# yyl404/NSGP-RePRE

Measured on NVIDIA B200. Metric: nsgp_cov_projection_throughput, higher is better.
Workload: dtype f32 (3xTF32 tensor-core products, fp32 accumulate)

## Files before the change

nsgp-repre_b200/csrc/api.cu:

```cuda
#include <cstdarg>
#include <mutex>
#include <vector>

#include "../../include/nsgp_repre_b200.h"
#include "common.cuh"
#include "geometry.h"
#include "repre.h"
#include "sgd.h"

namespace nsgp {

static thread_local char g_err[512] = "";
unsigned long long g_launches = 0;
#ifdef NSGP_BRINGUP
int g_engine = 0;
#endif

int g_profile = 0;
namespace {
struct ProfRec { cudaEvent_t a, b; };
std::vector<ProfRec> g_prof[kProfKinds];
cudaEvent_t g_prof_open[kProfKinds];
}
namespace {
// ... 1137 lines not shown
               "kmeans_assign: workspace too small");
  size_t n8 = (size_t)round_up(n, 8), k8 = (size_t)round_up(k, 8);
  char* ws = align_up((char*)workspace, 1024);
  float* xh = reinterpret_cast<float*>(ws);
  float* xl = xh + n8 * D;
  float* ch = xl + n8 * D;
  float* cl = ch + k8 * D;
  float* dots = cl + k8 * D;
  int ld = (int)round_up(k, 4);
  float* cn = dots + n8 * ld;
  int rc = launch_split(X, xh, xl, (long long)n * D, stream);
  if (rc) return rc;
  rc = launch_split(centres, ch, cl, (long long)k * D, stream);
  if (rc) return rc;
  rc = launch_row_sqnorm(centres, k, D, D, cn, stream);
  if (rc) return rc;
  NSGP_CHECK_CUDA(cudaMemsetAsync(dots, 0, (size_t)n * ld * 4, stream));
  ContractionArgs a{};
  a.A = matrix_operand(xh, xl, n, D, D);
  a.B = matrix_operand(ch, cl, k, D, D);
  a.out = dots;
  a.ld = ld;
  a.n_cols = k;
  a.alpha = 1.f;
  a.epi = kEpiGemmRmw;
  a.splits = 1;
  rc = contraction(a, stream);
  if (rc) return rc;
  return launch_kmeans_argmin(dots, n, k, ld, cn, (long long*)labels, stream);
}

#ifdef NSGP_BRINGUP
int nsgp_debug_read_counters(unsigned long long* out, int n) {
  NSGP_REQUIRE(out && n != 0 && n <= 160 * 8 && n >= -160 * 8, "debug_read_counters: bad arguments");
  if (n < 0) return debug_read_ac_counters(out, -n);
  return debug_read_counters(out, n);
}

int nsgp_debug_mma_rate(int mode, int iters, unsigned long long* out_dev, int n_ctas,
                        void* stream_) {
  NSGP_REQUIRE(out_dev && iters > 0 && n_ctas > 0, "debug_mma_rate: bad arguments");
  return debug_mma_rate(mode, iters, out_dev, n_ctas, (cudaStream_t)stream_);
}

int nsgp_debug_timeline_read(unsigned long long* out, int* kinds, int max_slots) {
  NSGP_REQUIRE(out && kinds && max_slots > 0, "timeline_read: bad arguments");
  NSGP_CHECK_CUDA(cudaDeviceSynchronize());
  const int n = g_tl_n < max_slots ? g_tl_n : max_slots;
  if (n > 0) {
    NSGP_CHECK_CUDA(cudaMemcpy(out, g_tl_dev, (size_t)n * 2 * sizeof(unsigned long long),
                               cudaMemcpyDeviceToHost));
    for (int i = 0; i < n; ++i) kinds[i] = g_tl_kind[i];
    std::vector<unsigned long long> init(kTlSlots * 2);
    for (int i = 0; i < kTlSlots; ++i) { init[2 * i] = ~0ull; init[2 * i + 1] = 0; }
    cudaMemcpy(g_tl_dev, init.data(), init.size() * sizeof(unsigned long long), cudaMemcpyHostToDevice);
  }
  g_tl_n = 0;
  return n;
}

int nsgp_debug_occupy(int threads, size_t smem, long long cycles, int n_ctas, void* stream_) {
  NSGP_REQUIRE(threads > 0 && threads <= 1024 && n_ctas > 0 && smem <= 227 * 1024,
               "debug_occupy: bad arguments");
  return debug_occupy(threads, smem, cycles, n_ctas, (cudaStream_t)stream_);
}

int nsgp_debug_tma3d_probe(const float* base, long long img_elems, int B, int box_rows,
// ... 45 lines not shown
```

nsgp-repre_b200/csrc/contraction_tc.cu:

```cuda
#include <algorithm>
#include <cstdlib>
#include <mutex>
#include <vector>
#include <unordered_map>

#include "common.cuh"
#include "tc_common.cuh"

namespace nsgp {

using namespace tc;

namespace {

constexpr int BN = 128;
constexpr int STAGES = 3;
constexpr uint32_t kABytes = BM * BK * 4;
constexpr uint32_t kStageBytes = 4 * kABytes;
constexpr uint32_t kTmemCols = 512;

__device__ __forceinline__ int seg_count(int r0, int rows, int br) {
  int n = 0;
  for (int r = r0; r < r0 + BM && r < rows; r += br) ++n;
  return n;
}

struct Item {
  const TcMaps* maps;
  const TcParams* p;
  int rb, cb, kb0, kb1;
};

__device__ __forceinline__ Item fetch_item(const TcMaps* pmaps, const TcParams* pp,
                                           const TcProblem* gprobs, const TcItem* gitems,
                                           int idx) {
  Item it;
  if (gitems != nullptr) {
    const int4 a = *reinterpret_cast<const int4*>(&gitems[idx]);
    const int kb1 = gitems[idx].kb1;
    it.maps = &gprobs[a.x].maps;
    it.p = &gprobs[a.x].p;
    it.rb = a.y; it.cb = a.z; it.kb0 = a.w; it.kb1 = kb1;
    return it;
  }
  it.maps = pmaps;
  it.p = pp;
  const int split = idx / pp->n_tiles;
  int tile = idx - split * pp->n_tiles;
  if (pp->gram) {
    int rb = 0;
    for (;; ++rb) {
      const int cnt = pp->tiles_n - rb;
      if (tile < cnt) break;
      tile -= cnt;
    }
    it.rb = rb; it.cb = rb + tile;
  } else {
    it.rb = tile / pp->tiles_n;
    it.cb = tile - it.rb * pp->tiles_n;
  }
  it.kb0 = (int)((long long)pp->nkb * split / pp->splits);
  it.kb1 = (int)((long long)pp->nkb * (split + 1) / pp->splits);
  return it;
}

__device__ unsigned long long g_dbg_counters[160 * 8];

template <bool PAIR>
__global__ void __launch_bounds__(kThreads, 1)
contraction_tc_kernel(const __grid_constant__ TcMaps pmaps, const __grid_constant__ TcParams pp,
                      const TcProblem* __restrict__ gprobs, const TcItem* __restrict__ gitems,
                      int n_items_max, int prefetch_dist, int dbg,
                      unsigned long long* tl, const int* __restrict__ n_items_dev) {
  const int n_items = n_items_dev != nullptr ? min(n_items_max, __ldg(n_items_dev)) : n_items_max;
  extern __shared__ __align__(1024) uint8_t smem_raw[];
  uint8_t* smem = reinterpret_cast<uint8_t*>(
      (reinterpret_cast<uintptr_t>(smem_raw) + 1023) & ~(uintptr_t)1023);
  uint64_t* full_bar = reinterpret_cast<uint64_t*>(smem + STAGES * kStageBytes);
  uint64_t* empty_bar = full_bar + STAGES;
  uint64_t* tmem_full = empty_bar + STAGES;
  uint64_t* tmem_empty = tmem_full + 2;
  uint64_t* peer_full = tmem_empty + 2;
  uint32_t* tmem_base_slot = reinterpret_cast<uint32_t*>(peer_full + STAGES);

  constexpr int TILE = PAIR ? 256 : 128;
  const int warp = threadIdx.x >> 5;
  const int lane = threadIdx.x & 31;
  const int rank = PAIR ? (int)cluster_ctarank() : 0;
  const int worker = PAIR ? (int)(blockIdx.x >> 1) : (int)blockIdx.x;
  const int n_workers = PAIR ? (int)(gridDim.x >> 1) : (int)gridDim.x;
  const long long t_start = clock64();
  asm volatile("griddepcontrol.launch_dependents;" ::: "memory");
  tl_begin(tl);
  long long c_wait = 0, c_issue = 0, c_acc = 0, c_kb = 0;

  if (warp == 0 && lane == 0) {
    for (int s = 0; s < STAGES; ++s) {
      mbar_init(&full_bar[s], 1);
      mbar_init(&empty_bar[s], 1);
      mbar_init(&peer_full[s], 1);
    }
    for (int b = 0; b < 2; ++b) {
      mbar_init(&tmem_full[b], 1);
      mbar_init(&tmem_empty[b], PAIR ? 8 : 4);
    }
    asm volatile("fence.mbarrier_init.release.cluster;" ::: "memory");
  }
  if (warp == 1) {
    if (PAIR) {
      asm volatile("tcgen05.alloc.cta_group::2.sync.aligned.shared::cta.b32 [%0], %1;" ::"r"(
                       smem_u32(tmem_base_slot)),
                   "r"(kTmemCols)
                   : "memory");
      asm volatile("tcgen05.relinquish_alloc_permit.cta_group::2.sync.aligned;" ::: "memory");
    } else {
      asm volatile("tcgen05.alloc.cta_group::1.sync.aligned.shared::cta.b32 [%0], %1;" ::"r"(
                       smem_u32(tmem_base_slot)),
                   "r"(kTmemCols)
                   : "memory");
      asm volatile("tcgen05.relinquish_alloc_permit.cta_group::1.sync.aligned;" ::: "memory");
    }
  }
  tc_fence_before();
  __syncthreads();
  if (PAIR) cluster_sync();
  tc_fence_after();
  const uint32_t tmem_base = *tmem_base_slot;

  if (warp == 0) {
    uint32_t stage = 0, phase = 0;
    int pf_idx = worker, pf_kb = 0;
    Item pf_it{};
    bool pf_live = prefetch_dist > 0 && pf_idx < n_items;
    if (pf_live) { pf_it = fetch_item(&pmaps, &pp, gprobs, gitems, pf_idx); pf_kb = pf_it.kb0; }
    auto prefetch_step = [&]() {
      if (!pf_live) return;
      const TcParams& q = *pf_it.p;
      const bool pa = q.gram ? (pf_it.rb == pf_it.cb) : (pf_it.cb == 0);
      const bool pb = q.gram ? false : (pf_it.rb == 0);
      const int kx = pf_kb * BK;
      if (pa) {
        const int r0 = pf_it.rb * TILE + rank * BM;
        for (int r = r0; r < r0 + BM && r < q.A.rows; r += q.A.br) {
          const int t = r / q.A.Cs, c = r - t * q.A.Cs;
          const int px = q.A.tile_nkb ? 0 : kx;
          const int py = q.A.tile_nkb ? (((c >> 7) * q.A.tile_nkb + pf_kb) << 7) + (c & 127) : c;
          tma_prefetch_2d_elect(&pf_it.maps->a[0][t], px, py);
          tma_prefetch_2d_elect(&pf_it.maps->a[1][t], px, py);
        }
      }
      if (pb) {
        const int c0 = pf_it.cb * TILE + rank * BM;
        for (int r = c0; r < c0 + BM && r < q.B.rows; r += q.B.br) {
          const int t = r / q.B.Cs, c = r - t * q.B.Cs;
          const int px = q.B.tile_nkb ? 0 : kx;
          const int py = q.B.tile_nkb ? (((c >> 7) * q.B.tile_nkb + pf_kb) << 7) + (c & 127) : c;
          tma_prefetch_2d_elect(&pf_it.maps->b[0][t], px, py);
          tma_prefetch_2d_elect(&pf_it.maps->b[1][t], px, py);
        }
      }
      if (++pf_kb >= pf_it.kb1) {
        pf_idx += n_workers;
        pf_live = pf_idx < n_items;
        if (pf_live) { pf_it = fetch_item(&pmaps, &pp, gprobs, gitems, pf_idx); pf_kb = pf_it.kb0; }
      }
    };
    for (int i = 0; i < prefetch_dist; ++i) prefetch_step();
    for (int idx = worker; idx < n_items; idx += n_workers) {
      const Item it = fetch_item(&pmaps, &pp, gprobs, gitems, idx);
      const TcParams& p = *it.p;
      const int r0 = it.rb * TILE + rank * BM;
      const int c0 = it.cb * TILE + rank * BM;
      const bool share = p.gram && p.same_operand && it.rb == it.cb;
      const int a_rows = p.A.rows, a_br = p.A.br, a_cs = p.A.Cs, a_tn = p.A.tile_nkb;
      const int b_rows = p.B.rows, b_br = p.B.br, b_cs = p.B.Cs, b_tn = p.B.tile_nkb;
      const int segs_a = seg_count(r0, a_rows, a_br);
      const int segs_b = share ? 0 : seg_count(c0, b_rows, b_br);
      const uint32_t tx =
          ((dbg & 4) ? 1u : 2u) * (uint32_t)(segs_a * a_br + segs_b * b_br) * BK * 4u;
      for (int kb = it.kb0; kb < it.kb1; ++kb) {
        prefetch_step();
        long long t0 = (dbg & 1) ? clock64() : 0;
        if (dbg & 8) mbar_wait(&empty_bar[stage], phase ^ 1);
        else mbar_wait_warp(&empty_bar[stage], phase ^ 1, lane);
        long long t1 = (dbg & 1) ? clock64() : 0;
        c_wait += t1 - t0;
        mbar_expect_tx_elect(&full_bar[stage], tx);
        const uint32_t sbase = smem_u32(smem + stage * kStageBytes);
        const int kx0 = kb * BK;
        for (int s = 0; s < segs_a; ++s) {
          const int r = r0 + s * a_br;
          const int t = r / a_cs, c = r - t * a_cs;
          const uint32_t off = (uint32_t)(s * a_br) * (BK * 4);
          const int lx = a_tn ? 0 : kx0;
          const int ly = a_tn ? (((c >> 7) * a_tn + kb) << 7) + (c & 127) : c;
          tma_load_2d_elect(sbase + off, &it.maps->a[0][t], &full_bar[stage], lx, ly);
          if (!(dbg & 4)) tma_load_2d_elect(sbase + kABytes + off, &it.maps->a[1][t], &full_bar[stage], lx, ly);
        }
        for (int s = 0; s < segs_b; ++s) {
          const int r = c0 + s * b_br;
          const int t = r / b_cs, c = r - t * b_cs;
          const uint32_t off = (uint32_t)(s * b_br) * (BK * 4);
          const int lx = b_tn ? 0 : kx0;
          const int ly = b_tn ? (((c >> 7) * b_tn + kb) << 7) + (c & 127) : c;
          tma_load_2d_elect(sbase + 2 * kABytes + off, &it.maps->b[0][t], &full_bar[stage], lx, ly);
          if (!(dbg & 4)) tma_load_2d_elect(sbase + 3 * kABytes + off, &it.maps->b[1][t], &full_bar[stage], lx, ly);
        }
        if (dbg & 1) c_issue += clock64() - t1;
        if (++stage == STAGES) { stage = 0; phase ^= 1; }
      }
    }
    if ((dbg & 1) && lane == 0) {
      g_dbg_counters[blockIdx.x * 8 + 3] = c_wait;
      g_dbg_counters[blockIdx.x * 8 + 4] = c_issue;
    }
  } else if (warp == 1) {
    if (!PAIR || rank == 0) {
      uint32_t stage = 0, phase = 0;
      uint32_t local_item = 0;
      for (int idx = worker; idx < n_items; idx += n_workers, ++local_item) {
        const Item it = fetch_item(&pmaps, &pp, gprobs, gitems, idx);
        const TcParams& p = *it.p;
        const bool share = p.gram && p.same_operand && it.rb == it.cb;
        int n_valid = p.n_cols - it.cb * TILE;
        if (n_valid > TILE) n_valid = TILE;
        const uint32_t idesc = PAIR ? make_idesc_tf32(256, 256)
                                    : make_idesc_tf32(BM, (n_valid + 15) & ~15);
        const uint32_t buf = local_item & 1;
        const uint32_t use = local_item >> 1;
        long long ta = (dbg & 1) ? clock64() : 0;
        mbar_wait_warp(&tmem_empty[buf], (use & 1) ^ 1, lane);
        if (dbg & 1) c_acc += clock64() - ta;
        tc_fence_after();
        const uint32_t d_main = tmem_base + buf * 256;
        const uint32_t d_corr = d_main + 128;
        for (int kb = it.kb0; kb < it.kb1; ++kb) {
          long long t0 = (dbg & 1) ? clock64() : 0;
          if (dbg & 8) mbar_wait(&full_bar[stage], phase);
          else mbar_wait_warp(&full_bar[stage], phase, lane);
          if (PAIR) mbar_wait_warp(&peer_full[stage], phase, lane);
          long long t1 = (dbg & 1) ? clock64() : 0;
          c_wait += t1 - t0;
          ++c_kb;
          tc_fence_after();
          const uint32_t sbase = smem_u32(smem + stage * kStageBytes);
          const uint64_t a_hi = make_kmajor_sw128_desc(sbase);
          const uint64_t a_lo = make_kmajor_sw128_desc(sbase + kABytes);
          const uint64_t b_hi = share ? a_hi : make_kmajor_sw128_desc(sbase + 2 * kABytes);
          const uint64_t b_lo = share ? a_lo : make_kmajor_sw128_desc(sbase + 3 * kABytes);
          const uint32_t first = kb > it.kb0 ? 1u : 0u;
          if (PAIR) {
            tc_mma_kblock_3xtf32_2sm(d_main, a_hi, a_lo, b_hi, b_lo, idesc, first);
            tc_commit_2sm_mc_elect(&empty_bar[stage]);
            if (kb == it.kb1 - 1) tc_commit_2sm_mc_elect(&tmem_full[buf]);
          } else {
            if (dbg & 2) tc_mma_kblock_3xtf32(d_main, d_corr, a_hi, a_hi, b_hi, b_hi, idesc, first, 2u);
            else tc_mma_kblock_3xtf32(d_main, d_corr, a_hi, a_lo, b_hi, b_lo, idesc, first, 0u);
            tc_commit_elect(&empty_bar[stage]);
            if (kb == it.kb1 - 1) tc_commit_elect(&tmem_full[buf]);
          }
          if (dbg & 1) c_issue += clock64() - t1;
          if (++stage == STAGES) { stage = 0; phase ^= 1; }
        }
        if (it.kb1 <= it.kb0) {
          if (PAIR) tc_commit_2sm_mc_elect(&tmem_full[buf]);
          else tc_commit_elect(&tmem_full[buf]);
        }
      }
      if ((dbg & 1) && lane == 0) {
        g_dbg_counters[blockIdx.x * 8 + 0] = c_wait;
        g_dbg_counters[blockIdx.x * 8 + 1] = c_issue;
        g_dbg_counters[blockIdx.x * 8 + 2] = c_acc;
        g_dbg_counters[blockIdx.x * 8 + 5] = clock64() - t_start;
        g_dbg_counters[blockIdx.x * 8 + 6] = c_kb;
      }
    } else {
      uint32_t stage = 0, phase = 0;
      for (int idx = worker; idx < n_items; idx += n_workers) {
        const Item it = fetch_item(&pmaps, &pp, gprobs, gitems, idx);
        for (int kb = it.kb0; kb < it.kb1; ++kb) {
          mbar_wait_warp(&full_bar[stage], phase, lane);
          mbar_arrive_remote_elect(&peer_full[stage], 0);
          if (++stage == STAGES) { stage = 0; phase ^= 1; }
        }
      }
    }
  } else {
    const int quad = warp & 3;
    uint32_t local_item = 0;
    for (int idx = worker; idx < n_items; idx += n_workers, ++local_item) {
      const Item it = fetch_item(&pmaps, &pp, gprobs, gitems, idx);
      const TcParams& p = *it.p;
      const uint32_t buf = local_item & 1;
      const uint32_t use = local_item >> 1;
      mbar_wait_warp(&tmem_full[buf], use & 1, lane, 200);
      tc_fence_after();
      const int rblk = it.rb * TILE + rank * BM;
      const int row = rblk + quad * 32 + lane;
      const bool row_ok = row < p.A.rows && it.kb1 > it.kb0;
      float* orow = p.out + (long long)row * p.ld;
      const float alpha = p.alpha;
      const int n_cols = p.n_cols;
      const bool vec = p.vec_red != 0;
      const bool gram = p.gram != 0;
#pragma unroll 1
      for (int chunk = 0; chunk < TILE / 32; ++chunk) {
        uint32_t v[32];
        const uint32_t taddr = tmem_base + ((uint32_t)(quad * 32) << 16) + buf * 256 + chunk * 32;
        tc_ld32(taddr, v);
        if (!PAIR) {
          uint32_t w[32];
          tc_ld32(taddr + 128, w);
          tc_wait_ld();
#pragma unroll
          for (int j = 0; j < 32; ++j)
            v[j] = __float_as_uint(__uint_as_float(v[j]) + __uint_as_float(w[j]));
        } else {
          tc_wait_ld();
        }
        const int col0 = it.cb * TILE + chunk * 32;
        const bool wanted = !gram || (col0 + 31 >= rblk);
        if (row_ok && col0 < n_cols && wanted) {
#pragma unroll
          for (int j = 0; j < 32; j += 4) {
            const int col = col0 + j;
            const float x0 = alpha * __uint_as_float(v[j]), x1 = alpha * __uint_as_float(v[j + 1]),
                        x2 = alpha * __uint_as_float(v[j + 2]), x3 = alpha * __uint_as_float(v[j + 3]);
            if (vec && col + 3 < n_cols) {
              red_add_v4(orow + col, x0, x1, x2, x3);
            } else {
              if (col < n_cols) atomicAdd(orow + col, x0);
              if (col + 1 < n_cols) atomicAdd(orow + col + 1, x1);
              if (col + 2 < n_cols) atomicAdd(orow + col + 2, x2);
              if (col + 3 < n_cols) atomicAdd(orow + col + 3, x3);
            }
          }
        }
      }
      tc_fence_before();
      __syncwarp();
      if (!PAIR || rank == 0) {
        if (lane == 0) mbar_arrive(&tmem_empty[buf]);
      } else {
        mbar_arrive_remote_elect(&tmem_empty[buf], 0);
      }
    }
  }

  tc_fence_before();
  __syncthreads();
  tl_end(tl);
  if (PAIR) cluster_sync();
  if (warp == 1) {
    tc_fence_after();
    if (PAIR)
      asm volatile("tcgen05.dealloc.cta_group::2.sync.aligned.b32 %0, %1;" ::"r"(tmem_base),
                   "r"(kTmemCols)
                   : "memory");
    else
      asm volatile("tcgen05.dealloc.cta_group::1.sync.aligned.b32 %0, %1;" ::"r"(tmem_base),
                   "r"(kTmemCols)
                   : "memory");
  }
}

typedef CUresult (*EncodeTiledFn)(CUtensorMap*, CUtensorMapDataType, cuuint32_t, void*,
                                  const cuuint64_t*, const cuuint64_t*, const cuuint32_t*,
                                  const cuuint32_t*, CUtensorMapInterleave, CUtensorMapSwizzle,
                                  CUtensorMapL2promotion, CUtensorMapFloatOOBfill);

EncodeTiledFn get_encode_fn() {
  static EncodeTiledFn fn = nullptr;
  static std::once_flag once;
  std::call_once(once, [] {
    void* p = nullptr;
    cudaDriverEntryPointQueryResult q;
    if (cudaGetDriverEntryPoint("cuTensorMapEncodeTiled", &p, cudaEnableDefault, &q) ==
            cudaSuccess &&
        q == cudaDriverEntryPointSuccess)
      fn = reinterpret_cast<EncodeTiledFn>(p);
  });
  return fn;
}

int pick_box_rows(const Operand& o) {
  if (o.T == 1) {
    int br = 128;
    while (br > o.Cs) br >>= 1;
    return br < 8 ? 0 : br;
  }
  for (int br = 128; br >= 8; br >>= 1)
    if (o.Cs % br == 0) return br;
  return 0;
}

int encode_operand(const Operand& o, int br, CUtensorMap (*dst)[kMaxTaps]) {
  EncodeTiledFn enc = get_encode_fn();
  NSGP_REQUIRE(enc != nullptr, "tcgen05 engine: cuTensorMapEncodeTiled is unavailable");
  for (int hl = 0; hl < 2; ++hl)
    for (int t = 0; t < o.T; ++t) {
      const float* base = o.base + (long long)hl * o.hl_stride + o.tap_off[t];
      NSGP_REQUIRE((reinterpret_cast<uintptr_t>(base) & 15) == 0,
                   "tcgen05 engine: operand base must be 16-byte aligned");
      cuuint64_t gdim[2] = {(cuuint64_t)o.K, (cuuint64_t)o.Cs};
      cuuint64_t gstr[1] = {(cuuint64_t)o.row_pitch * 4};
      if (o.tile_nkb > 0) {
        gdim[0] = BK;
        gdim[1] = (cuuint64_t)ceil_div(o.Cs, 128) * o.tile_nkb * 128;
        gstr[0] = BK * 4;
      }
      cuuint32_t box[2] = {(cuuint32_t)BK, (cuuint32_t)br};
      cuuint32_t estr[2] = {1, 1};
      CUresult r = enc(&dst[hl][t], CU_TENSOR_MAP_DATA_TYPE_FLOAT32, 2, (void*)base, gdim, gstr,
                       box, estr, CU_TENSOR_MAP_INTERLEAVE_NONE, CU_TENSOR_MAP_SWIZZLE_128B,
                       CU_TENSOR_MAP_L2_PROMOTION_L2_256B, CU_TENSOR_MAP_FLOAT_OOB_FILL_NONE);
      NSGP_REQUIRE(r == CUDA_SUCCESS,
                   "cuTensorMapEncodeTiled failed (%d): K=%d Cs=%d pitch=%lld br=%d", (int)r, o.K,
                   o.Cs, o.row_pitch, br);
    }
  return 0;
}

void fill_operand(const Operand& o, int br, TcOperand* d) {
  d->T = o.T; d->Cs = o.Cs; d->rows = o.rows; d->br = br;
  d->tile_nkb = o.tile_nkb; d->pad0 = d->pad1 = d->pad2 = 0;
}

constexpr size_t kSmemBytes = (size_t)STAGES * kStageBytes + 1024 + 256;
constexpr size_t kSmemBytesFullSm = (size_t)7 * 32768 + 1024 + 256;

int dbg_counters() {
  static const int d = (nsgp_env("NSGP_DBG_COUNTERS") ? 1 : 0) | (nsgp_env("NSGP_DBG_MMA2") ? 2 : 0) |
                       (nsgp_env("NSGP_DBG_HALFLOAD") ? 4 : 0) | (nsgp_env("NSGP_DBG_ALLPOLL") ? 8 : 0);
  return d;
}

int prefetch_distance() {
  static const int d = [] {
    const char* e = nsgp_env("NSGP_PREFETCH");
    return e ? atoi(e) : 8;
  }();
  return d;
}

template <bool PAIR>
int configure_kernel() {
  static bool configured = false;
// ... 95 lines not shown
  NSGP_REQUIRE(br_a > 0 && br_b > 0, "tcgen05 engine: operand rows per tap must be >= 8 "
               "(multiple of 8 when taps > 1)");
  TcParams& p = out->p;
  p = TcParams{};
  p.nkb = k_blocks(a.A);
  if (a.A.rows == 0 || a.n_cols == 0 || p.nkb == 0) return 1;
  int rc = encode_operand(a.A, br_a, out->maps.a);
  if (rc) return rc;
  rc = encode_operand(a.B, br_b, out->maps.b);
  if (rc) return rc;
  fill_operand(a.A, br_a, &p.A);
  fill_operand(a.B, br_b, &p.B);
  p.out = a.out; p.ld = a.ld; p.n_cols = a.n_cols; p.alpha = a.alpha;
  p.gram = (a.epi == kEpiGramAtomic) ? 1 : 0;
  p.same_operand = (p.gram && a.A.base == a.B.base && a.A.hl_stride == a.B.hl_stride &&
                    a.A.rows == a.B.rows) ? 1 : 0;
  p.pair = pair ? 1 : 0;
  p.chain = a.chain;
  const int tile = pair ? 256 : 128;
  p.tiles_m = ceil_div(a.A.rows, tile);
  p.tiles_n = ceil_div(a.n_cols, tile);
  NSGP_REQUIRE(!p.gram || p.tiles_m == p.tiles_n, "Gram: operands must have the same rows");
  p.n_tiles = p.gram ? p.tiles_m * (p.tiles_m + 1) / 2 : p.tiles_m * p.tiles_n;
  static const int vec_red = [] {
    const char* e = nsgp_env("NSGP_VEC_RED");
    return (e && e[0] == '0') ? 0 : 1;
  }();
  p.vec_red = (vec_red && a.ld % 4 == 0 && (reinterpret_cast<uintptr_t>(a.out) & 15) == 0) ? 1 : 0;
  p.splits = 1;
  return 0;
}

int chain_limit(const TcParams& p) {
  static const int gram_chain = [] {
    const char* e = nsgp_env("NSGP_CHAIN");
    return e ? atoi(e) : kChainGram;
  }();
  if (p.chain > 0) return p.pair && p.chain > 32 ? 32 : p.chain;
  if (!p.gram) return kChainGemm;
  return p.pair ? 32 : gram_chain;
}

}

int encode_batch_rows_map(CUtensorMap* dst, const float* base, long long img_elems, int B,
                          int box_rows) {
  EncodeTiledFn enc = get_encode_fn();
  NSGP_REQUIRE(enc != nullptr, "cuTensorMapEncodeTiled is unavailable");
  NSGP_REQUIRE(img_elems % 256 == 0 && (reinterpret_cast<uintptr_t>(base) & 15) == 0,
               "batch rows map: input must be 16-byte aligned with a multiple of 256 elements");
  cuuint64_t gdim[3] = {256, (cuuint64_t)(img_elems / 256), (cuuint64_t)B};
  cuuint64_t gstr[2] = {1024, (cuuint64_t)img_elems * 4};
  cuuint32_t box[3] = {256, (cuuint32_t)box_rows, (cuuint32_t)B};
  cuuint32_t estr[3] = {1, 1, 1};
  CUresult r = enc(dst, CU_TENSOR_MAP_DATA_TYPE_FLOAT32, 3, (void*)base, gdim, gstr, box, estr,
                   CU_TENSOR_MAP_INTERLEAVE_NONE, CU_TENSOR_MAP_SWIZZLE_NONE,
                   CU_TENSOR_MAP_L2_PROMOTION_L2_256B, CU_TENSOR_MAP_FLOAT_OOB_FILL_NONE);
  NSGP_REQUIRE(r == CUDA_SUCCESS, "cuTensorMapEncodeTiled (batch rows) failed (%d)", (int)r);
  return 0;
}

namespace tc {
int sm_count() {
  static int n = 0;
  if (n == 0) {
    int dev = 0;
    cudaGetDevice(&dev);
    cudaDeviceGetAttribute(&n, cudaDevAttrMultiProcessorCount, dev);
    if (n <= 0) n = 148;
  }
  return n;
}
}
// ... 164 lines not shown
```

nsgp-repre_b200/csrc/tc_common.cuh:

```cuda
#pragma once
#include "common.cuh"

namespace nsgp {
namespace tc {

constexpr int BM = 128;
constexpr int BK = 32;
constexpr int UMMA_K = 8;
constexpr int kThreads = 192;
constexpr int kEpiWarp0 = 2;

struct alignas(64) TcMaps {
  CUtensorMap a[2][kMaxTaps];
  CUtensorMap b[2][kMaxTaps];
};

struct TcOperand {
  int T, Cs, rows, br;
  int tile_nkb, pad0, pad1, pad2;
};

struct TcParams {
  TcOperand A, B;
  float* out;
// ... 91 lines not shown
      "tcgen05.mma.cta_group::1.kind::tf32 [%0], %1, %2, %3, p;\n\t}" ::"r"(d_tmem),
      "l"(adesc), "l"(bdesc), "r"(idesc), "r"(accumulate)
      : "memory");
}
__device__ __forceinline__ void tc_ld32(uint32_t taddr, uint32_t (&v)[32]) {
  asm volatile(
      "tcgen05.ld.sync.aligned.32x32b.x32.b32 "
      "{%0, %1, %2, %3, %4, %5, %6, %7, %8, %9, %10, %11, %12, %13, %14, %15, "
      "%16, %17, %18, %19, %20, %21, %22, %23, %24, %25, %26, %27, %28, %29, %30, %31}, [%32];"
      : "=r"(v[0]), "=r"(v[1]), "=r"(v[2]), "=r"(v[3]), "=r"(v[4]), "=r"(v[5]), "=r"(v[6]),
        "=r"(v[7]), "=r"(v[8]), "=r"(v[9]), "=r"(v[10]), "=r"(v[11]), "=r"(v[12]), "=r"(v[13]),
        "=r"(v[14]), "=r"(v[15]), "=r"(v[16]), "=r"(v[17]), "=r"(v[18]), "=r"(v[19]),
        "=r"(v[20]), "=r"(v[21]), "=r"(v[22]), "=r"(v[23]), "=r"(v[24]), "=r"(v[25]),
        "=r"(v[26]), "=r"(v[27]), "=r"(v[28]), "=r"(v[29]), "=r"(v[30]), "=r"(v[31])
      : "r"(taddr)
      : "memory");
}
__device__ __forceinline__ void tc_wait_ld() {
  asm volatile("tcgen05.wait::ld.sync.aligned;" ::: "memory");
}
__device__ __forceinline__ void red_add_v4(float* p, float a, float b, float c, float d) {
  asm volatile("red.global.add.v4.f32 [%0], {%1, %2, %3, %4};" ::"l"(p), "f"(a), "f"(b),
               "f"(c), "f"(d)
               : "memory");
}

__device__ __forceinline__ uint64_t make_kmajor_sw128_desc(uint32_t saddr) {
  uint64_t d = 0;
  d |= (uint64_t)((saddr >> 4) & 0x3FFF);
  d |= (uint64_t)1 << 16;
  d |= (uint64_t)(1024 >> 4) << 32;
  d |= (uint64_t)1 << 46;
  d |= (uint64_t)2 << 61;
  return d;
}

__host__ __device__ constexpr uint32_t make_idesc_tf32(int M, int N) {
  return (1u << 4) | (2u << 7) | (2u << 10) | ((uint32_t)(N >> 3) << 17) |
         ((uint32_t)(M >> 4) << 24);
}


__device__ __forceinline__ void mbar_expect_tx_elect(uint64_t* bar, uint32_t bytes) {
  asm volatile(
      "{\n\t.reg .pred pe;\n\t"
      "elect.sync _|pe, 0xffffffff;\n\t"
      "@pe mbarrier.arrive.expect_tx.shared::cta.b64 _, [%0], %1;\n\t}" ::"r"(smem_u32(bar)),
      "r"(bytes)
      : "memory");
}
__device__ __forceinline__ void tma_load_2d_elect(uint32_t dst, const CUtensorMap* map,
                                                  uint64_t* bar, int x, int c) {
  asm volatile(
      "{\n\t.reg .pred pe;\n\t"
      "elect.sync _|pe, 0xffffffff;\n\t"
      "@pe cp.async.bulk.tensor.2d.shared::cluster.global.tile.mbarrier::complete_tx::bytes "
      "[%0], [%1, {%3, %4}], [%2];\n\t}" ::"r"(dst),
      "l"(reinterpret_cast<uint64_t>(map)), "r"(smem_u32(bar)), "r"(x), "r"(c)
      : "memory");
}
__device__ __forceinline__ void tc_commit_elect(uint64_t* bar) {
  asm volatile(
      "{\n\t.reg .pred pe;\n\t"
      "elect.sync _|pe, 0xffffffff;\n\t"
      "@pe tcgen05.commit.cta_group::1.mbarrier::arrive::one.shared::cluster.b64 [%0];\n\t}" ::
      "r"(smem_u32(bar))
// ... 8 lines not shown
      ".reg .pred pe, pf, pc, pt;\n\t"
      "setp.eq.b32 pt, 0, 0;\n\t"
      ".reg .b64 ah, al, bh, bl;\n\t"
      "elect.sync _|pe, 0xffffffff;\n\t"
      "setp.ne.b32 pf, %7, 0;\n\t"
      "setp.eq.b32 pc, %8, 1;\n\t"
      "or.pred pc, pc, pf;\n\t"
      ".reg .pred ps, pq;\n\t"
      "setp.lt.u32 ps, %8, 2;\n\t"
      "and.pred ps, ps, pe;\n\t"
      "setp.ne.b32 pq, %8, 3;\n\t"
      "and.pred pq, pq, pe;\n\t"
      "@pe tcgen05.mma.cta_group::1.kind::tf32 [%0], %2, %4, %6, pf;\n\t"
      "@pq tcgen05.mma.cta_group::1.kind::tf32 [%1], %3, %4, %6, pc;\n\t"
      "@ps tcgen05.mma.cta_group::1.kind::tf32 [%1], %2, %5, %6, pt;\n\t"
      "add.u64 ah, %2, 2; add.u64 al, %3, 2; add.u64 bh, %4, 2; add.u64 bl, %5, 2;\n\t"
      "@pe tcgen05.mma.cta_group::1.kind::tf32 [%0], ah, bh, %6, pt;\n\t"
      "@pq tcgen05.mma.cta_group::1.kind::tf32 [%1], al, bh, %6, pt;\n\t"
      "@ps tcgen05.mma.cta_group::1.kind::tf32 [%1], ah, bl, %6, pt;\n\t"
      "add.u64 ah, %2, 4; add.u64 al, %3, 4; add.u64 bh, %4, 4; add.u64 bl, %5, 4;\n\t"
      "@pe tcgen05.mma.cta_group::1.kind::tf32 [%0], ah, bh, %6, pt;\n\t"
      "@pq tcgen05.mma.cta_group::1.kind::tf32 [%1], al, bh, %6, pt;\n\t"
      "@ps tcgen05.mma.cta_group::1.kind::tf32 [%1], ah, bl, %6, pt;\n\t"
      "add.u64 ah, %2, 6; add.u64 al, %3, 6; add.u64 bh, %4, 6; add.u64 bl, %5, 6;\n\t"
      "@pe tcgen05.mma.cta_group::1.kind::tf32 [%0], ah, bh, %6, pt;\n\t"
      "@pq tcgen05.mma.cta_group::1.kind::tf32 [%1], al, bh, %6, pt;\n\t"
      "@ps tcgen05.mma.cta_group::1.kind::tf32 [%1], ah, bl, %6, pt;\n\t"
      "}" ::"r"(d_main),
      "r"(d_corr), "l"(a_hi), "l"(a_lo), "l"(b_hi), "l"(b_lo), "r"(idesc), "r"(first),
      "r"(same_acc)
      : "memory");
}

__device__ __forceinline__ void tc_cp_a_kblock(uint32_t t_hi, uint32_t t_lo, uint64_t a_hi,
                                               uint64_t a_lo) {
  asm volatile(
      "{\n\t.reg .pred pe;\n\t.reg .b64 ah, al;\n\t"
      "elect.sync _|pe, 0xffffffff;\n\t"
      "@pe tcgen05.cp.cta_group::1.128x256b [%0], %2;\n\t"
      "@pe tcgen05.cp.cta_group::1.128x256b [%1], %3;\n\t"
      "add.u64 ah, %2, 2; add.u64 al, %3, 2;\n\t"
      "@pe tcgen05.cp.cta_group::1.128x256b [%0 + 8], ah;\n\t"
      "@pe tcgen05.cp.cta_group::1.128x256b [%1 + 8], al;\n\t"
      "add.u64 ah, %2, 4; add.u64 al, %3, 4;\n\t"
      "@pe tcgen05.cp.cta_group::1.128x256b [%0 + 16], ah;\n\t"
      "@pe tcgen05.cp.cta_group::1.128x256b [%1 + 16], al;\n\t"
      "add.u64 ah, %2, 6; add.u64 al, %3, 6;\n\t"
      "@pe tcgen05.cp.cta_group::1.128x256b [%0 + 24], ah;\n\t"
      "@pe tcgen05.cp.cta_group::1.128x256b [%1 + 24], al;\n\t"
      "}" ::"r"(t_hi), "r"(t_lo), "l"(a_hi), "l"(a_lo)
      : "memory");
}
__device__ __forceinline__ void tc_mma_kblock_3xtf32_ta(uint32_t d, uint32_t t_hi, uint32_t t_lo,
                                                        uint64_t b_hi, uint64_t b_lo,
                                                        uint32_t idesc, uint32_t first) {
  asm volatile(
      "{\n\t"
      ".reg .pred pe, pf, pt;\n\t"
      ".reg .b64 bh, bl;\n\t"
      "setp.eq.b32 pt, 0, 0;\n\t"
      "elect.sync _|pe, 0xffffffff;\n\t"
      "setp.ne.b32 pf, %6, 0;\n\t"
      "@pe tcgen05.mma.cta_group::1.kind::tf32 [%0], [%1], %3, %5, pf;\n\t"
      "@pe tcgen05.mma.cta_group::1.kind::tf32 [%0], [%2], %3, %5, pt;\n\t"
      "@pe tcgen05.mma.cta_group::1.kind::tf32 [%0], [%1], %4, %5, pt;\n\t"
      "add.u64 bh, %3, 2; add.u64 bl, %4, 2;\n\t"
// ... 42 lines not shown
      "r"(rank)
      : "memory");
}
__device__ __forceinline__ void tc_mma_kblock_3xtf32_2sm(uint32_t d, uint64_t a_hi, uint64_t a_lo,
                                                         uint64_t b_hi, uint64_t b_lo,
                                                         uint32_t idesc, uint32_t first) {
  asm volatile(
      "{\n\t"
      ".reg .pred pe, pf, pt;\n\t"
      ".reg .b64 ah, al, bh, bl;\n\t"
      "setp.eq.b32 pt, 0, 0;\n\t"
      "elect.sync _|pe, 0xffffffff;\n\t"
      "setp.ne.b32 pf, %6, 0;\n\t"
      "@pe tcgen05.mma.cta_group::2.kind::tf32 [%0], %2, %3, %5, pf;\n\t"
      "@pe tcgen05.mma.cta_group::2.kind::tf32 [%0], %1, %4, %5, pt;\n\t"
      "@pe tcgen05.mma.cta_group::2.kind::tf32 [%0], %1, %3, %5, pt;\n\t"
      "add.u64 ah, %1, 2; add.u64 al, %2, 2; add.u64 bh, %3, 2; add.u64 bl, %4, 2;\n\t"
      "@pe tcgen05.mma.cta_group::2.kind::tf32 [%0], al, bh, %5, pt;\n\t"
      "@pe tcgen05.mma.cta_group::2.kind::tf32 [%0], ah, bl, %5, pt;\n\t"
      "@pe tcgen05.mma.cta_group::2.kind::tf32 [%0], ah, bh, %5, pt;\n\t"
      "add.u64 ah, %1, 4; add.u64 al, %2, 4; add.u64 bh, %3, 4; add.u64 bl, %4, 4;\n\t"
      "@pe tcgen05.mma.cta_group::2.kind::tf32 [%0], al, bh, %5, pt;\n\t"
      "@pe tcgen05.mma.cta_group::2.kind::tf32 [%0], ah, bl, %5, pt;\n\t"
      "@pe tcgen05.mma.cta_group::2.kind::tf32 [%0], ah, bh, %5, pt;\n\t"
      "add.u64 ah, %1, 6; add.u64 al, %2, 6; add.u64 bh, %3, 6; add.u64 bl, %4, 6;\n\t"
      "@pe tcgen05.mma.cta_group::2.kind::tf32 [%0], al, bh, %5, pt;\n\t"
      "@pe tcgen05.mma.cta_group::2.kind::tf32 [%0], ah, bl, %5, pt;\n\t"
      "@pe tcgen05.mma.cta_group::2.kind::tf32 [%0], ah, bh, %5, pt;\n\t"
      "}" ::"r"(d),
      "l"(a_hi), "l"(a_lo), "l"(b_hi), "l"(b_lo), "r"(idesc), "r"(first)
      : "memory");
}

__device__ __forceinline__ void tma_prefetch_2d_elect(const CUtensorMap* map, int x, int c) {
  asm volatile(
      "{\n\t.reg .pred pe;\n\t"
      "elect.sync _|pe, 0xffffffff;\n\t"
      "@pe cp.async.bulk.prefetch.tensor.2d.L2.global.tile [%0, {%1, %2}];\n\t}" ::"l"(
          reinterpret_cast<uint64_t>(map)),
      "r"(x), "r"(c)
      : "memory");
}

constexpr uint32_t kPeerBitMask = 0xFEFFFFFFu;
__device__ __forceinline__ uint32_t cluster_ctarank() {
  uint32_t r;
  asm volatile("mov.u32 %0, %%cluster_ctarank;" : "=r"(r));
  return r;
}
__device__ __forceinline__ void cluster_sync() {
  asm volatile("barrier.cluster.arrive.release.aligned;" ::: "memory");
  asm volatile("barrier.cluster.wait.acquire.aligned;" ::: "memory");
}
__device__ __forceinline__ void mbar_arrive_remote(uint64_t* bar, uint32_t rank) {
  asm volatile(
      "{\n\t.reg .b32 ra;\n\t"
      "mapa.shared::cluster.u32 ra, %0, %1;\n\t"
      "mbarrier.arrive.release.cluster.shared::cluster.b64 _, [ra];\n\t}" ::"r"(smem_u32(bar)),
      "r"(rank)
      : "memory");
}
__device__ __forceinline__ void tma_load_2d_2sm(uint32_t dst, const CUtensorMap* map,
                                                uint64_t* bar, int x, int c) {
  asm volatile(
      "cp.async.bulk.tensor.2d.cta_group::2.shared::cluster.global.mbarrier::complete_tx::bytes "
      "[%0], [%1, {%3, %4}], [%2];" ::"r"(dst),
// ... 27 lines not shown
```

Measured before the change: 433.1.

## Split k-blocks into half-width SW64 stages and deepen pipeline to seven

```diff
diff --git a/nsgp-repre_b200/csrc/api.cu b/nsgp-repre_b200/csrc/api.cu
--- a/nsgp-repre_b200/csrc/api.cu
+++ b/nsgp-repre_b200/csrc/api.cu
@@ -1193,7 +1193,7 @@
 
 #ifdef NSGP_BRINGUP
 int nsgp_debug_read_counters(unsigned long long* out, int n) {
-  NSGP_REQUIRE(out && n != 0 && n <= 160 * 8 && n >= -160 * 8, "debug_read_counters: bad arguments");
+  NSGP_REQUIRE(out && n != 0 && n <= 2 * 160 * 8 && n >= -160 * 8, "debug_read_counters: bad arguments");
   if (n < 0) return debug_read_ac_counters(out, -n);
   return debug_read_counters(out, n);
 }
diff --git a/nsgp-repre_b200/csrc/contraction_tc.cu b/nsgp-repre_b200/csrc/contraction_tc.cu
--- a/nsgp-repre_b200/csrc/contraction_tc.cu
+++ b/nsgp-repre_b200/csrc/contraction_tc.cu
@@ -14,8 +14,10 @@
 namespace {
 
 constexpr int BN = 128;
-constexpr int STAGES = 3;
-constexpr uint32_t kABytes = BM * BK * 4;
+constexpr int SUB = 2;
+constexpr int BKS = BK / SUB;
+constexpr int STAGES = 7;
+constexpr uint32_t kABytes = BM * BKS * 4;
 constexpr uint32_t kStageBytes = 4 * kABytes;
 constexpr uint32_t kTmemCols = 512;
 
@@ -64,7 +66,7 @@
   return it;
 }
 
-__device__ unsigned long long g_dbg_counters[160 * 8];
+__device__ unsigned long long g_dbg_counters[2 * 160 * 8];
 
 template <bool PAIR>
 __global__ void __launch_bounds__(kThreads, 1)
@@ -73,6 +75,9 @@
                       int n_items_max, int prefetch_dist, int dbg,
                       unsigned long long* tl, const int* __restrict__ n_items_dev) {
   const int n_items = n_items_dev != nullptr ? min(n_items_max, __ldg(n_items_dev)) : n_items_max;
+#ifndef NSGP_BRINGUP
+  dbg = 0;
+#endif
   extern __shared__ __align__(1024) uint8_t smem_raw[];
   uint8_t* smem = reinterpret_cast<uint8_t*>(
       (reinterpret_cast<uintptr_t>(smem_raw) + 1023) & ~(uintptr_t)1023);
@@ -92,7 +97,7 @@
   const long long t_start = clock64();
   asm volatile("griddepcontrol.launch_dependents;" ::: "memory");
   tl_begin(tl);
-  long long c_wait = 0, c_issue = 0, c_acc = 0, c_kb = 0;
+  long long c_wait = 0, c_issue = 0, c_acc = 0, c_kb = 0, c_peer = 0;
 
   if (warp == 0 && lane == 0) {
     for (int s = 0; s < STAGES; ++s) {
@@ -145,8 +150,10 @@
           const int t = r / q.A.Cs, c = r - t * q.A.Cs;
           const int px = q.A.tile_nkb ? 0 : kx;
           const int py = q.A.tile_nkb ? (((c >> 7) * q.A.tile_nkb + pf_kb) << 7) + (c & 127) : c;
-          tma_prefetch_2d_elect(&pf_it.maps->a[0][t], px, py);
-          tma_prefetch_2d_elect(&pf_it.maps->a[1][t], px, py);
+          for (int h = 0; h < SUB; ++h) {
+            tma_prefetch_2d_elect(&pf_it.maps->a[0][t], px + h * BKS, py);
+            tma_prefetch_2d_elect(&pf_it.maps->a[1][t], px + h * BKS, py);
+          }
         }
       }
       if (pb) {
@@ -155,8 +162,10 @@
           const int t = r / q.B.Cs, c = r - t * q.B.Cs;
           const int px = q.B.tile_nkb ? 0 : kx;
           const int py = q.B.tile_nkb ? (((c >> 7) * q.B.tile_nkb + pf_kb) << 7) + (c & 127) : c;
-          tma_prefetch_2d_elect(&pf_it.maps->b[0][t], px, py);
-          tma_prefetch_2d_elect(&pf_it.maps->b[1][t], px, py);
+          for (int h = 0; h < SUB; ++h) {
+            tma_prefetch_2d_elect(&pf_it.maps->b[0][t], px + h * BKS, py);
+            tma_prefetch_2d_elect(&pf_it.maps->b[1][t], px + h * BKS, py);
+          }
         }
       }
       if (++pf_kb >= pf_it.kb1) {
@@ -177,9 +186,10 @@
       const int segs_a = seg_count(r0, a_rows, a_br);
       const int segs_b = share ? 0 : seg_count(c0, b_rows, b_br);
       const uint32_t tx =
-          ((dbg & 4) ? 1u : 2u) * (uint32_t)(segs_a * a_br + segs_b * b_br) * BK * 4u;
-      for (int kb = it.kb0; kb < it.kb1; ++kb) {
-        prefetch_step();
+          ((dbg & 4) ? 1u : 2u) * (uint32_t)(segs_a * a_br + segs_b * b_br) * BKS * 4u;
+      for (int j = it.kb0 * SUB; j < it.kb1 * SUB; ++j) {
+        const int kb = j / SUB, h = j - kb * SUB;
+        if (h == 0) prefetch_step();
         long long t0 = (dbg & 1) ? clock64() : 0;
         if (dbg & 8) mbar_wait(&empty_bar[stage], phase ^ 1);
         else mbar_wait_warp(&empty_bar[stage], phase ^ 1, lane);
@@ -187,12 +197,12 @@
         c_wait += t1 - t0;
         mbar_expect_tx_elect(&full_bar[stage], tx);
         const uint32_t sbase = smem_u32(smem + stage * kStageBytes);
-        const int kx0 = kb * BK;
+        const int kx0 = kb * BK + h * BKS;
         for (int s = 0; s < segs_a; ++s) {
           const int r = r0 + s * a_br;
           const int t = r / a_cs, c = r - t * a_cs;
-          const uint32_t off = (uint32_t)(s * a_br) * (BK * 4);
-          const int lx = a_tn ? 0 : kx0;
+          const uint32_t off = (uint32_t)(s * a_br) * (BKS * 4);
+          const int lx = a_tn ? h * BKS : kx0;
           const int ly = a_tn ? (((c >> 7) * a_tn + kb) << 7) + (c & 127) : c;
           tma_load_2d_elect(sbase + off, &it.maps->a[0][t], &full_bar[stage], lx, ly);
           if (!(dbg & 4)) tma_load_2d_elect(sbase + kABytes + off, &it.maps->a[1][t], &full_bar[stage], lx, ly);
@@ -200,8 +210,8 @@
         for (int s = 0; s < segs_b; ++s) {
           const int r = c0 + s * b_br;
           const int t = r / b_cs, c = r - t * b_cs;
-          const uint32_t off = (uint32_t)(s * b_br) * (BK * 4);
-          const int lx = b_tn ? 0 : kx0;
+          const uint32_t off = (uint32_t)(s * b_br) * (BKS * 4);
+          const int lx = b_tn ? h * BKS : kx0;
           const int ly = b_tn ? (((c >> 7) * b_tn + kb) << 7) + (c & 127) : c;
           tma_load_2d_elect(sbase + 2 * kABytes + off, &it.maps->b[0][t], &full_bar[stage], lx, ly);
           if (!(dbg & 4)) tma_load_2d_elect(sbase + 3 * kABytes + off, &it.maps->b[1][t], &full_bar[stage], lx, ly);
@@ -234,30 +244,33 @@
         tc_fence_after();
         const uint32_t d_main = tmem_base + buf * 256;
         const uint32_t d_corr = d_main + 128;
-        for (int kb = it.kb0; kb < it.kb1; ++kb) {
+        for (int j = it.kb0 * SUB; j < it.kb1 * SUB; ++j) {
           long long t0 = (dbg & 1) ? clock64() : 0;
           if (dbg & 8) mbar_wait(&full_bar[stage], phase);
           else mbar_wait_warp(&full_bar[stage], phase, lane);
+          long long tp = (dbg & 1) ? clock64() : 0;
           if (PAIR) mbar_wait_warp(&peer_full[stage], phase, lane);
           long long t1 = (dbg & 1) ? clock64() : 0;
-          c_wait += t1 - t0;
-          ++c_kb;
+          c_wait += tp - t0;
+          c_peer += t1 - tp;
+          if (j % SUB == 0) ++c_kb;
           tc_fence_after();
           const uint32_t sbase = smem_u32(smem + stage * kStageBytes);
-          const uint64_t a_hi = make_kmajor_sw128_desc(sbase);
-          const uint64_t a_lo = make_kmajor_sw128_desc(sbase + kABytes);
-          const uint64_t b_hi = share ? a_hi : make_kmajor_sw128_desc(sbase + 2 * kABytes);
-          const uint64_t b_lo = share ? a_lo : make_kmajor_sw128_desc(sbase + 3 * kABytes);
-          const uint32_t first = kb > it.kb0 ? 1u : 0u;
+          const uint64_t a_hi = make_kmajor_sw64_desc(sbase);
+          const uint64_t a_lo = make_kmajor_sw64_desc(sbase + kABytes);
+          const uint64_t b_hi = share ? a_hi : make_kmajor_sw64_desc(sbase + 2 * kABytes);
+          const uint64_t b_lo = share ? a_lo : make_kmajor_sw64_desc(sbase + 3 * kABytes);
+          const uint32_t first = j > it.kb0 * SUB ? 1u : 0u;
+          const bool last = j == it.kb1 * SUB - 1;
           if (PAIR) {
-            tc_mma_kblock_3xtf32_2sm(d_main, a_hi, a_lo, b_hi, b_lo, idesc, first);
+            tc_mma_half_3xtf32_2sm(d_main, a_hi, a_lo, b_hi, b_lo, idesc, first);
             tc_commit_2sm_mc_elect(&empty_bar[stage]);
-            if (kb == it.kb1 - 1) tc_commit_2sm_mc_elect(&tmem_full[buf]);
+            if (last) tc_commit_2sm_mc_elect(&tmem_full[buf]);
           } else {
-            if (dbg & 2) tc_mma_kblock_3xtf32(d_main, d_corr, a_hi, a_hi, b_hi, b_hi, idesc, first, 2u);
-            else tc_mma_kblock_3xtf32(d_main, d_corr, a_hi, a_lo, b_hi, b_lo, idesc, first, 0u);
+            if (dbg & 2) tc_mma_half_3xtf32(d_main, d_corr, a_hi, a_hi, b_hi, b_hi, idesc, first, 2u);
+            else tc_mma_half_3xtf32(d_main, d_corr, a_hi, a_lo, b_hi, b_lo, idesc, first, 0u);
             tc_commit_elect(&empty_bar[stage]);
-            if (kb == it.kb1 - 1) tc_commit_elect(&tmem_full[buf]);
+            if (last) tc_commit_elect(&tmem_full[buf]);
           }
           if (dbg & 1) c_issue += clock64() - t1;
           if (++stage == STAGES) { stage = 0; phase ^= 1; }
@@ -273,12 +286,13 @@
         g_dbg_counters[blockIdx.x * 8 + 2] = c_acc;
         g_dbg_counters[blockIdx.x * 8 + 5] = clock64() - t_start;
         g_dbg_counters[blockIdx.x * 8 + 6] = c_kb;
+        g_dbg_counters[blockIdx.x * 8 + 7] = c_peer;
       }
     } else {
       uint32_t stage = 0, phase = 0;
       for (int idx = worker; idx < n_items; idx += n_workers) {
         const Item it = fetch_item(&pmaps, &pp, gprobs, gitems, idx);
-        for (int kb = it.kb0; kb < it.kb1; ++kb) {
+        for (int j = it.kb0 * SUB; j < it.kb1 * SUB; ++j) {
           mbar_wait_warp(&full_bar[stage], phase, lane);
           mbar_arrive_remote_elect(&peer_full[stage], 0);
           if (++stage == STAGES) { stage = 0; phase ^= 1; }
@@ -293,7 +307,10 @@
       const TcParams& p = *it.p;
       const uint32_t buf = local_item & 1;
       const uint32_t use = local_item >> 1;
+      const long long te0 = (dbg & 1) ? clock64() : 0;
       mbar_wait_warp(&tmem_full[buf], use & 1, lane, 200);
+      const long long te1 = (dbg & 1) ? clock64() : 0;
+      c_wait += te1 - te0;
       tc_fence_after();
       const int rblk = it.rb * TILE + rank * BM;
       const int row = rblk + quad * 32 + lane;
@@ -344,6 +361,11 @@
       } else {
         mbar_arrive_remote_elect(&tmem_empty[buf], 0);
       }
+      if (dbg & 1) c_issue += clock64() - te1;
+    }
+    if ((dbg & 1) && warp == kEpiWarp0 && lane == 0) {
+      g_dbg_counters[160 * 8 + blockIdx.x * 8 + 0] = c_wait;
+      g_dbg_counters[160 * 8 + blockIdx.x * 8 + 1] = c_issue;
     }
   }
 
@@ -409,10 +431,10 @@
         gdim[1] = (cuuint64_t)ceil_div(o.Cs, 128) * o.tile_nkb * 128;
         gstr[0] = BK * 4;
       }
-      cuuint32_t box[2] = {(cuuint32_t)BK, (cuuint32_t)br};
+      cuuint32_t box[2] = {(cuuint32_t)BKS, (cuuint32_t)br};
       cuuint32_t estr[2] = {1, 1};
       CUresult r = enc(&dst[hl][t], CU_TENSOR_MAP_DATA_TYPE_FLOAT32, 2, (void*)base, gdim, gstr,
-                       box, estr, CU_TENSOR_MAP_INTERLEAVE_NONE, CU_TENSOR_MAP_SWIZZLE_128B,
+                       box, estr, CU_TENSOR_MAP_INTERLEAVE_NONE, CU_TENSOR_MAP_SWIZZLE_64B,
                        CU_TENSOR_MAP_L2_PROMOTION_L2_256B, CU_TENSOR_MAP_FLOAT_OOB_FILL_NONE);
       NSGP_REQUIRE(r == CUDA_SUCCESS,
                    "cuTensorMapEncodeTiled failed (%d): K=%d Cs=%d pitch=%lld br=%d", (int)r, o.K,
@@ -574,13 +596,14 @@
 }
 
 int chain_limit(const TcParams& p) {
-  static const int gram_chain = [] {
+  static const int chain_env = [] {
     const char* e = nsgp_env("NSGP_CHAIN");
-    return e ? atoi(e) : kChainGram;
+    return e ? atoi(e) : 0;
   }();
   if (p.chain > 0) return p.pair && p.chain > 32 ? 32 : p.chain;
   if (!p.gram) return kChainGemm;
-  return p.pair ? 32 : gram_chain;
+  if (chain_env > 0) return chain_env;
+  return p.pair ? 32 : kChainGram;
 }
 
 }
diff --git a/nsgp-repre_b200/csrc/tc_common.cuh b/nsgp-repre_b200/csrc/tc_common.cuh
--- a/nsgp-repre_b200/csrc/tc_common.cuh
+++ b/nsgp-repre_b200/csrc/tc_common.cuh
@@ -147,6 +147,16 @@
   d |= (uint64_t)(1024 >> 4) << 32;
   d |= (uint64_t)1 << 46;
   d |= (uint64_t)2 << 61;
+  return d;
+}
+
+__device__ __forceinline__ uint64_t make_kmajor_sw64_desc(uint32_t saddr) {
+  uint64_t d = 0;
+  d |= (uint64_t)((saddr >> 4) & 0x3FFF);
+  d |= (uint64_t)1 << 16;
+  d |= (uint64_t)(512 >> 4) << 32;
+  d |= (uint64_t)1 << 46;
+  d |= (uint64_t)4 << 61;
   return d;
 }
 
@@ -221,6 +231,37 @@
       : "memory");
 }
 
+__device__ __forceinline__ void tc_mma_half_3xtf32(uint32_t d_main, uint32_t d_corr,
+                                                   uint64_t a_hi, uint64_t a_lo, uint64_t b_hi,
+                                                   uint64_t b_lo, uint32_t idesc,
+                                                   uint32_t first, uint32_t same_acc) {
+  asm volatile(
+      "{\n\t"
+      ".reg .pred pe, pf, pc, pt;\n\t"
+      "setp.eq.b32 pt, 0, 0;\n\t"
+      ".reg .b64 ah, al, bh, bl;\n\t"
+      "elect.sync _|pe, 0xffffffff;\n\t"
+      "setp.ne.b32 pf, %7, 0;\n\t"
+      "setp.eq.b32 pc, %8, 1;\n\t"
+      "or.pred pc, pc, pf;\n\t"
+      ".reg .pred ps, pq;\n\t"
+      "setp.lt.u32 ps, %8, 2;\n\t"
+      "and.pred ps, ps, pe;\n\t"
+      "setp.ne.b32 pq, %8, 3;\n\t"
+      "and.pred pq, pq, pe;\n\t"
+      "@pe tcgen05.mma.cta_group::1.kind::tf32 [%0], %2, %4, %6, pf;\n\t"
+      "@pq tcgen05.mma.cta_group::1.kind::tf32 [%1], %3, %4, %6, pc;\n\t"
+      "@ps tcgen05.mma.cta_group::1.kind::tf32 [%1], %2, %5, %6, pt;\n\t"
+      "add.u64 ah, %2, 2; add.u64 al, %3, 2; add.u64 bh, %4, 2; add.u64 bl, %5, 2;\n\t"
+      "@pe tcgen05.mma.cta_group::1.kind::tf32 [%0], ah, bh, %6, pt;\n\t"
+      "@pq tcgen05.mma.cta_group::1.kind::tf32 [%1], al, bh, %6, pt;\n\t"
+      "@ps tcgen05.mma.cta_group::1.kind::tf32 [%1], ah, bl, %6, pt;\n\t"
+      "}" ::"r"(d_main),
+      "r"(d_corr), "l"(a_hi), "l"(a_lo), "l"(b_hi), "l"(b_lo), "r"(idesc), "r"(first),
+      "r"(same_acc)
+      : "memory");
+}
+
 __device__ __forceinline__ void tc_cp_a_kblock(uint32_t t_hi, uint32_t t_lo, uint64_t a_hi,
                                                uint64_t a_lo) {
   asm volatile(
@@ -329,6 +370,28 @@
       : "memory");
 }
 
+__device__ __forceinline__ void tc_mma_half_3xtf32_2sm(uint32_t d, uint64_t a_hi, uint64_t a_lo,
+                                                       uint64_t b_hi, uint64_t b_lo,
+                                                       uint32_t idesc, uint32_t first) {
+  asm volatile(
+      "{\n\t"
+      ".reg .pred pe, pf, pt;\n\t"
+      ".reg .b64 ah, al, bh, bl;\n\t"
+      "setp.eq.b32 pt, 0, 0;\n\t"
+      "elect.sync _|pe, 0xffffffff;\n\t"
+      "setp.ne.b32 pf, %6, 0;\n\t"
+      "@pe tcgen05.mma.cta_group::2.kind::tf32 [%0], %2, %3, %5, pf;\n\t"
+      "@pe tcgen05.mma.cta_group::2.kind::tf32 [%0], %1, %4, %5, pt;\n\t"
+      "@pe tcgen05.mma.cta_group::2.kind::tf32 [%0], %1, %3, %5, pt;\n\t"
+      "add.u64 ah, %1, 2; add.u64 al, %2, 2; add.u64 bh, %3, 2; add.u64 bl, %4, 2;\n\t"
+      "@pe tcgen05.mma.cta_group::2.kind::tf32 [%0], al, bh, %5, pt;\n\t"
+      "@pe tcgen05.mma.cta_group::2.kind::tf32 [%0], ah, bl, %5, pt;\n\t"
+      "@pe tcgen05.mma.cta_group::2.kind::tf32 [%0], ah, bh, %5, pt;\n\t"
+      "}" ::"r"(d),
+      "l"(a_hi), "l"(a_lo), "l"(b_hi), "l"(b_lo), "r"(idesc), "r"(first)
+      : "memory");
+}
+
 __device__ __forceinline__ void tma_prefetch_2d_elect(const CUtensorMap* map, int x, int c) {
   asm volatile(
       "{\n\t.reg .pred pe;\n\t"
```

Result: slower. 383.3 (median of 6 runs) (-11.5%).
